# fenghansen/YOND_public

Hardware: AMD Instinct MI355X
Metric: Bayer megapixels/sec end-to-end (NLE+VST+denoise+iVST) (higher is better)
Workload: dtype f32 (3x3 convolutions: f32 operands as two f16 halves -- 22-23 significant bits -- on the f16 MFMA, 3 products per f32 product, f32 accumulate; per-layer error vs float64 asserted <= 2x the f32 direct kernel's and <= 2e-5 of max|ref| (tests/test_hip_conv.py; measured 1.3e-6 vs 1.5e-6), whole frame v

## Files before the change

### yond_public_amd/csrc/conv_split.hip

```cpp
#include "conv_split_kernel.h"

SPLIT_GROUP_K1S2(SPLIT_EXTERN)
SPLIT_GROUP_S1_64(SPLIT_EXTERN)
SPLIT_GROUP_S1_32(SPLIT_EXTERN)
SPLIT_GROUP_HALF(SPLIT_EXTERN)
SPLIT_GROUP_HALF128(SPLIT_EXTERN)
SPLIT_GROUP_HALF_TALL(SPLIT_EXTERN)
SPLIT_GROUP_FOLD(SPLIT_EXTERN)
SPLIT_GROUP_FOLD_S2(SPLIT_EXTERN)
SPLIT_GROUP_FOLD_K1(SPLIT_EXTERN)
SPLIT_GROUP_FOLD_NHWC(SPLIT_EXTERN)
SPLIT_GROUP_K1_D2(SPLIT_EXTERN)
SPLIT_GROUP_OSP(SPLIT_EXTERN)
SPLIT_GROUP_ISP(SPLIT_EXTERN)
SPLIT_GROUP_ISP_OSP(SPLIT_EXTERN)
SPLIT_GROUP_ISP_K1S2(SPLIT_EXTERN)
SPLIT_GROUP_K1_SUB2(SPLIT_EXTERN)
SPLIT_GROUP_WRES(SPLIT_EXTERN)
SPLIT_GROUP_D2(SPLIT_EXTERN)
SPLIT_GROUP_H_OSP(SPLIT_EXTERN)
SPLIT_GROUP_H_ISP_OSP(SPLIT_EXTERN)
SPLIT_GROUP_H_ISP_O4(SPLIT_EXTERN)
SPLIT_GROUP_H_K1S2(SPLIT_EXTERN)
SPLIT_GROUP_H_D2(SPLIT_EXTERN)
SPLIT_GROUP_H_SUB2(SPLIT_EXTERN)
SPLIT_GROUP_H128_OSP(SPLIT_EXTERN)
SPLIT_GROUP_H128_ISP_OSP(SPLIT_EXTERN)
// ... 180 lines not shown
            if (!isp || !d.src1) return YOND_EUNSUPPORTED;
            if (half128k1) return launch_split<1, 8, 128, 2, 1, 3, false, false, true, 2>(d, st);
            if (d.dst2) return launch_split<1, 8, 64, 2, 1, 3, false, false, true, 2, false, false, true>(d, st);
            if (tn == 64 && op4 && (long long)(d.Cout / 64) * ((d.Wo + 31) / 32) * ((d.Ho + 15) / 16) * d.N >= 256 && yond_exp_long("YOND_SPLIT_K1_TALL", 1) != 0)
                return launch_split<1, 16, 64, 4, 1, 2, false, false, true, 2>(d, st);
            return tn == 32 ? launch_split<1, 8, 32, 1, 1, 3, false, false, true, 2>(d, st) : launch_split<1, 8, 64, 2, 1, 3, false, false, true, 2>(d, st);
        }
        if (isp && tn == 64 && d.Wo <= 16 && d.src1 && !d.dst2 && yond_exp_long("YOND_SPLIT_FOLD", 1) != 0) {
            const int f = d.Wo <= 8 ? 4 : 2;
            const long long subs = (long long)d.N * ((d.Ho + 7) / 8) * ((d.Wo + 32 / f - 1) / (32 / f));
            const long long tiles_f = (long long)(d.Cout / 64) * ((subs + f - 1) / f), tiles = (long long)(d.Cout / 64) * ((d.Ho + 7) / 8) * d.N;
            const bool fits = (long long)d.H * d.W * (d.C0 > 4 * d.C1 ? d.C0 : 4 * d.C1) * 4 * f < (1LL << 31);
            if (fits && (tiles_f + 255) / 256 < (tiles + 255) / 256)
                return f == 2 ? launch_split<1, 8, 64, 2, 2, 3, false, false, true, 2, false, false, false, 2>(d, st) : launch_split<1, 8, 64, 2, 2, 3, false, false, true, 2, false, false, false, 4>(d, st);
        }
        if (isp && d.dst2) return launch_split<1, 8, 64, 2, 2, 3, false, false, true, 2, false, false, true>(d, st);
        if (isp) return tn == 32 ? launch_split<1, 8, 32, 1, 2, 3, false, false, true, 2>(d, st) : launch_split<1, 8, 64, 2, 2, 3, false, false, true, 2>(d, st);
        if (tn == 32) return launch_split<1, 8, 32, 1, 2, 3, false, false, true>(d, st);
        return launch_split<1, 8, 64, 2, 2, 3, false, false, true>(d, st);
    }
    if (d.stride == 2) {
        if (d.Ho != (d.H + 1) / 2 || d.Wo != (d.W + 1) / 2 || d.pre_act) return YOND_EINVAL;
        if (osp || ip4 || (op4 && d.res)) return YOND_EUNSUPPORTED;
        if (isp && parts == 2 && d.Wo <= 16 && !d.src1 && !d.res && yond_exp_long("YOND_SPLIT_FOLD", 1) != 0) {
            const int f = d.Wo <= 8 ? 4 : 2;
            const long long subs = (long long)d.N * ((d.Ho + 3) / 4) * ((d.Wo + 32 / f - 1) / (32 / f));
            const long long tiles_f = (long long)(d.Cout / 64) * ((subs + f - 1) / f), tiles = (long long)(d.Cout / 64) * ((d.Ho + 3) / 4) * d.N;
            const bool fits = (long long)d.H * d.W * d.C0 * 4 * f < (1LL << 31);
            if (fits && (tiles_f + 255) / 256 < (tiles + 255) / 256) {
                if (f == 2) return d.dst2 ? launch_split<2, 4, 64, 1, 2, 2, false, false, false, 2, false, false, true, 2>(d, st) : launch_split<2, 4, 64, 1, 2, 2, false, false, false, 2, false, false, false, 2>(d, st);
// ... 131 lines not shown
```

### yond_public_amd/csrc/conv_split_kernel.h

```cpp
#pragma once
#include "common.h"
#include <cstdlib>

typedef _Float16 f16x8 __attribute__((ext_vector_type(8)));
typedef _Float16 f16x4 __attribute__((ext_vector_type(4)));

#ifndef SPLIT_DBG
#define SPLIT_DBG 0
#endif
#if SPLIT_DBG
static __device__ unsigned long long g_split_dbg[2][64][12];
#ifdef SPLIT_DBG_READER
extern "C" int SPLIT_DBG_READER(unsigned long long* host) {
    return (int)hipMemcpyFromSymbol(host, HIP_SYMBOL(g_split_dbg), sizeof(g_split_dbg));
}
#endif
#define SDBG(slot)                                                                                  \
    do {                                                                                            \
        if (blockIdx.x == 0 && (wave == 0 || wave == 4) && lane == 0 && dbg_step < 64)              \
            g_split_dbg[wave >> 2][dbg_step][slot] = __builtin_readcyclecounter();                  \
    } while (0)
#else
#define SDBG(slot) do {} while (0)
#endif
// ... 57 lines not shown
    return n;
}
__device__ __forceinline__ float split_silu(float x) {
    return x * __builtin_amdgcn_rcpf(1.0f + __builtin_amdgcn_exp2f(x * -1.44269504088896341f));
}
template <int N>
__device__ __forceinline__ void split_barrier_keep_loads() { asm volatile("s_waitcnt vmcnt(%0) lgkmcnt(0)\n\ts_barrier" ::"n"(N) : "memory"); }

template <int STRIDE, int TH, int TN, int MW, int PARTS, int NWB, bool PRE, bool O4 = false, bool K1 = false, int ISPM = 0, bool OSP = false, bool S2 = false, bool D2 = false, int FOLD = 0, int NWAVE = 8, int ROLES = 0>
__global__ __launch_bounds__(64 * NWAVE, (NWAVE == 4 && STRIDE == 1) ? 2 : 1) void conv_split_kernel(const YondConvDesc d) {
    using C = SplitCfg<STRIDE, TH, TN, MW, PARTS, NWB, K1, FOLD, NWAVE, ROLES>;
    static_assert(!ROLES || (ISPM == 2 && !OSP && !O4 && !PRE), "role split: the register-staged split-plane input (stride 2)");
    static_assert(!FOLD || (!O4 && !S2 && ((!K1 && STRIDE == 1 && ISPM != 2 && OSP) || (STRIDE == 2 && (ISPM == 2 || (ISPM == 0 && !PRE && !D2))) || (K1 && ISPM == 2) || (!K1 && STRIDE == 1 && ISPM == 0 && !OSP && !PRE))),
                  "folded tiles: the split-plane data flow's kernels (3x3 stride 1: LDS-DMA or register-staged input, split-plane store; stride 2 and the decoder GEMM: register-staged split planes) "
                  "and the plain [N][H][W][C] 3x3 layer (training, UNetSeeInDark)");
    constexpr bool ISP = ISPM == 1, ISR = ISPM == 2;
    static_assert(ISPM == 0 || !PRE, "split-plane input: the producer applied the activation");
    static_assert(!OSP || (!O4 && !K1 && STRIDE == 1), "split-plane output: 3x3 stride-1 layers");
    static_assert(!S2 || (K1 && ISPM == 2 && TN == 64), "two sub-positions per tile: the decoder GEMM with register-staged split planes");
    static_assert(!D2 || (!OSP && !O4 && ((!K1 && STRIDE == 2) || (K1 && ISPM == 2 && !S2 && TN == 64))), "second output: the stride-2 layers and the decoder GEMM at split precision");
    constexpr int NACC = PARTS;
    constexpr int IPP = ISR ? 2 * PARTS : 4;
    constexpr int PIX_ITEMS = C::IH * C::IW * IPP;
    constexpr int NITEM = C::NPT * PIX_ITEMS;
    static_assert(!K1 || PIX_ITEMS % C::NTS == 0, "1x1 mode: whole chunks per pass of the staging threads");
    constexpr int NIN = ISP ? 0 : (NITEM + C::NTS - 1) / C::NTS;
    constexpr int NINA = NIN > 0 ? NIN : 1;
    constexpr int NDI = ISP ? C::NDI : 0;
    constexpr int KD = K1 ? PIX_ITEMS / C::NTS : NIN;
    constexpr int DPER = C::WPP / split_gcd(C::WPP, NWAVE);
    constexpr int NG = ISP ? (NDI < DPER ? NDI : DPER) : KD;
    constexpr int NOPS = C::NWT + NIN + NDI;
    constexpr int KEEP = (ISP || ROLES) ? (C::WAHEAD == 2 ? C::NWT_MIN : 0) : (C::WAHEAD == 2 ? NIN + C::NWT_MIN : NIN);
    extern __shared__ __attribute__((aligned(16))) float smem[];

    const int tid = threadIdx.x, lane = tid & 63, wave = tid >> 6;
    const int stid = ROLES ? tid - C::NTS : tid;
    const bool consumer = !ROLES || __builtin_amdgcn_readfirstlane(wave) < C::NWC;
    const int li = lane & 31, lh = lane >> 5;
    constexpr int FSW = FOLD ? 32 / FOLD : 32;
    const int fsub = FOLD ? li / FSW : 0, fcol = FOLD ? li % FSW : li, flds = (FOLD && !K1) ? li + (STRIDE == 2 ? 1 : 2) * fsub : li;
    const int rg = wave % C::RG, cg = wave / C::RG;

    const int nct = d.Cout / TN;
    const bool computes = d.Cout > 0;
    const int fnsx = (d.Wo + FSW - 1) / FSW, fnsy = (d.Ho + TH - 1) / TH;
    const int fper = fnsy * fnsx, fsubs = d.N * fper;
    struct FGeo { int n, oy0, ox0; };
// ... 18 lines not shown
    const int Cr = K1 ? d.Cout / 4 : d.Cout;
    const int cpb = S2 ? Cr / 32 : 1;
    auto k1_sp = [&](int ct, int cu) -> int {
        if constexpr (S2) return 2 * (ct / cpb) + ((cu >> 5) & 1);
        return cu / Cr;
    };
    auto k1_cb = [&](int ct, int cu) -> int {
        if constexpr (S2) return (ct % cpb) * 32 + (cu & 31);
        return cu % Cr;
    };
    const int my_sl = stid & (IPP - 1);
    const int my_plane = (my_sl >> 1) * PARTS * C::PLANE + (my_sl & 1) * 2;

    int in_lds[NINA];
#pragma unroll
    for (int k = 0; k < NIN; ++k) {
        const int it = stid + k * C::NTS;
        const int pt = it / PIX_ITEMS;
        const int pix = (it % PIX_ITEMS) / IPP;
        const int py = pix / C::IW, px = pix % C::IW;
        const int lp = (STRIDE == 2) ? py * C::TWP + (px & 1) * C::HALF + (px >> 1) : py * C::TWP + px;
        in_lds[k] = my_plane + (it < NITEM ? pt * 2 * PARTS * C::PLANE + lp * 4 : C::IH * C::TWP * 4);
        if constexpr (ISR) in_lds[k] = my_sl * C::PLANE + (it < NITEM ? pt * 2 * PARTS * C::PLANE + lp * 4 : C::IH * C::TWP * 4);
    }

    struct Tile {
        int ct, n, ox0, oy0;
        int fu0;
        int goff[NG];
        int goff1[K1 ? NG : 1];
    };
// ... 21 lines not shown
    auto tile_origin = [&](const Cur& c, Tile& T) {
        T.n = rev ? Neff - 1 - c.n : c.n;
        T.ct = c.ct;
        T.ox0 = (rev ? ntx - 1 - c.tx : c.tx) * 32;
        T.oy0 = (rev ? nty - 1 - c.ty : c.ty) * TH;
        T.fu0 = 0;
        if constexpr (FOLD != 0) {
            T.fu0 = FOLD * (rev ? ntx - 1 - c.tx : c.tx);
            const FGeo g = fold_geo(T.fu0);
            T.n = g.n; T.oy0 = g.oy0; T.ox0 = g.ox0;
        }
    };
    auto decode = [&](const Cur& c, Tile& T) {
        tile_origin(c, T);
        const int n = T.n;
        if constexpr (ISP) {
#pragma unroll
            for (int k = 0; k < NG; ++k) {
                const int sid = k * NWAVE + wave_s;
                const int q = (sid % C::WPP) * 64 + lane;
                const int py = q / C::TWP, rem = q % C::TWP;
                const int px = STRIDE == 2 ? 2 * (rem % C::HALF) + rem / C::HALF : rem;
                const bool valid = q < C::UPP && px < C::IW;
                int gy = K1 ? T.oy0 + py : T.oy0 * STRIDE - 1 + py, gx = K1 ? T.ox0 + px : T.ox0 * STRIDE - 1 + px;
                int nshift = 0;
                if constexpr (FOLD != 0) {
                    const int sb = px / C::FSUBW, lx = px - C::FSUBW * sb;
                    const FGeo g = fold_geo(T.fu0 + sb);
                    gy = g.oy0 >= d.Ho ? -1 : g.oy0 - 1 + py;
                    gx = g.ox0 - 1 + lx;
                    nshift = (g.n - T.n) * ((d.C0 / 16) * (2 * PARTS) * PS0 * 16);
// ... 26 lines not shown
                nb = d.in_fmt == YOND_FMT_PLANES4 ? nb + (g.n - n) * (d.C0 / 4) * d.H * d.W : g.n * d.H * d.W;
                ushift = (g.n - n) * (d.C0 / 16) * (2 * PARTS) * PS0;
            }
            const bool ok = it < NITEM && gy >= 0 && gy < d.H && gx >= 0 && gx < d.W;
            T.goff[k] = ok ? (nb + gy * d.W + gx) : -1;
            if constexpr (ISR) T.goff[k] = ok ? gy * d.W + gx + ushift : d.H * d.W;
            if constexpr (K1) {
                const int sp = k1_sp(T.ct, T.ct * TN);
                T.goff1[k] = ok ? ((n * 2 * d.H + 2 * gy + (sp >> 1)) * (2 * d.W) + 2 * gx + (sp & 1)) : -1;
                if constexpr (ISR) T.goff1[k] = ok ? (2 * gy + (sp >> 1)) * (2 * d.W) + 2 * gx + (sp & 1) + ushift1 : 4 * d.H * d.W;
            }
        }
        }
    };

    constexpr int NSET = ROLES ? 1 : (MW >= 3 || (STRIDE == 2 && PARTS == 1 && TN == 128)) ? 2 : 3;
    static_assert(NSET == 3 || C::WAHEAD == 1, "the two-set pipeline goes with two weight buffers");
    f32x4 vin[NSET][NINA];
    unsigned vin_ok[NSET] = {};
    YondRange amax;
    struct LoadSrc { const float* src[C::NPT]; int A[C::NPT], B[C::NPT]; bool hi[C::NPT]; int dx[C::NPT]; };
    const bool in_p4 = d.in_fmt == YOND_FMT_PLANES4;
    auto load_src = [&](int ch, int n) {
        LoadSrc L;
#pragma unroll
        for (int t = 0; t < C::NPT; ++t) {
            const int c0 = (ch * C::NPT + t) * C::KC;
            const bool second = c0 >= d.C0;
            int Cs = second ? d.C1 : d.C0, cc = second ? c0 - d.C0 : c0;
            L.src[t] = second ? d.src1 : d.src0;
            L.hi[t] = second && K1;
            L.dx[t] = 0;
// ... 72 lines not shown
        const int plane = sid / C::WPP, wv = sid - plane * C::WPP;
        const int pt = plane / (2 * PARTS), pl = plane - pt * (2 * PARTS);
        const bool hi = K1 && ((I.hi >> pt) & 1u);
        const unsigned lds0 = (unsigned)(uintptr_t)(__attribute__((address_space(3))) float*)ob;
        const unsigned lds_wave = __builtin_amdgcn_readfirstlane(lds0 + (unsigned)(plane * C::PLANE * 4 + wv * 1024));
        const char* b0 = I.base[0];
        if constexpr (C::NPT > 1) b0 = pt == 1 ? I.base[1] : (pt == 2 ? I.base[C::NPT - 1] : b0);
        const unsigned long long ga = (unsigned long long)(uintptr_t)(b0 + (size_t)pl * (size_t)(hi ? PS1 : PS0) * 16);
        const unsigned ga_lo = __builtin_amdgcn_readfirstlane((unsigned)ga), ga_hi = __builtin_amdgcn_readfirstlane((unsigned)(ga >> 32));
        const char* gb = (const char*)(uintptr_t)(((unsigned long long)ga_hi << 32) | ga_lo);
        int voff = T.goff[k % NG];
        if constexpr (K1) voff = hi ? T.goff1[k % NG] : voff;
        if (sid < C::NDS && voff >= 0)
            asm volatile("s_mov_b32 m0, %0\n\ts_nop 0\n\tglobal_load_lds_dwordx4 %1, %2" ::"s"(lds_wave), "v"(voff), "s"(gb) : "memory");
    };
    auto weight_src = [&](int ct, int ch) {
        const unsigned long long a = (unsigned long long)(uintptr_t)(d.wpk + ((size_t)ct * nchunk + ch) * C::W_FLOATS);
        const unsigned lo = __builtin_amdgcn_readfirstlane((unsigned)a), hi = __builtin_amdgcn_readfirstlane((unsigned)(a >> 32));
        return (const float*)(uintptr_t)(((unsigned long long)hi << 32) | lo);
    };
    constexpr int NE = 4 * NIN;
    auto stage_task = [&](auto pc, auto ec, float* ob) {
        constexpr int P = decltype(pc)::value;
        constexpr int e = decltype(ec)::value, k = e / 4, j = e % 4;
        if constexpr (ISR) {
            if constexpr (j == 3) *(f32x4*)(ob + in_lds[k]) = vin[P][k];
            return;
        }
        float x = vin[P][k][j];
        if (PRE) x = split_silu(x);
        vin[P][k][j] = ((vin_ok[P] >> k) & 1u) ? x : 0.0f;
        if constexpr (j == 3) {
            const f32x4 v = vin[P][k];
            amax.add(v);
            const f16x4 h = {(_Float16)v[0], (_Float16)v[1], (_Float16)v[2], (_Float16)v[3]};
            *(f16x4*)(ob + in_lds[k]) = h;
// ... 42 lines not shown
            constexpr int po = K1 ? dx * 2 * PARTS * C::PLANE : 0;
#pragma unroll
            for (int p = 0; p < PARTS; ++p) xr[q % XD][p] = *(lds_h8)(xb + po + p * C::PLANE + (r * C::TWP + xo) * 4);
        };
        auto loadW1 = [&](auto dc, auto yc) {
            constexpr int dx = decltype(dc)::value, dy = decltype(yc)::value;
            constexpr int tap = K1 ? dx : dy * 3 + dx;
#pragma unroll
            for (int nn = 0; nn < C::NW; ++nn)
#pragma unroll
                for (int p = 0; p < PARTS; ++p)
                    wt[dx % WS][dy][nn][p] = *(lds_h8)(wb + ((tap * 2 * PARTS + p) * TN + nn * 32) * 4);
        };
        auto loadW = [&](auto dc) { static_for<0, (K1 ? 1 : 3)>([&](auto yc) { loadW1(dc, yc); }); };
        loadW(IntC<0>{});
        loadX(IntC<0>{});
        loadX(IntC<1>{});
        static_for<0, NQ>([&](auto qc) {
            constexpr int q = decltype(qc)::value;
            constexpr int dx = q / R, r = q % R;
            constexpr bool wpre = !WINPLACE && (r == (R >= 4 ? R - 3 : 0) && dx < 2);
            constexpr int wdy = r - (MW - 1) * STRIDE;
            constexpr bool wrep = WINPLACE && dx < 2 && wdy >= 0 && wdy <= 2;
            if constexpr (q + 2 < NQ) loadX(IntC<q + 2>{});
            if constexpr (wpre) loadW(IntC<dx + 1>{});
            constexpr int nmf = (PARTS == 2 ? 3 : 1) * C::NW * (K1 ? 1 : split_pairs(MW, STRIDE, r));
#pragma unroll
            for (int a = 0; a < 3; ++a) {
                if (PARTS == 1 && a != 1) continue;
#pragma unroll
                for (int m = 0; m < MW; ++m) {
                    const int dy = K1 ? (m == r ? 0 : -1) : r - m * STRIDE;
                    if (dy < 0 || dy > 2) continue;
#pragma unroll
                    for (int nn = 0; nn < C::NW; ++nn)
                        acc[a == 1 ? 0 : 1][m][nn] = __builtin_amdgcn_mfma_f32_32x32x16_f16(
                            wt[dx % WS][dy][nn][a == 2 ? PARTS - 1 : 0], xr[q % XD][a == 0 ? PARTS - 1 : 0], acc[a == 1 ? 0 : 1][m][nn], 0, 0, 0);
                }
            }
            if constexpr (wrep) loadW1(IntC<dx + 1>{}, IntC<wdy>{});
            if constexpr (q == 0) { if (wave_hi) __builtin_amdgcn_s_setprio(1); }
            if constexpr (q == NQ / 2) { if (wave_hi) __builtin_amdgcn_s_setprio(0); }
            if constexpr (q == Q0 - 1 && !ROLES) prep();
            if constexpr (q == NQ / 4) SDBG(8);
            if constexpr (q == NQ / 2) SDBG(9);
            if constexpr (q == (3 * NQ) / 4) SDBG(10);
            constexpr int qq = q >= Q0 ? q - Q0 : 0;
            constexpr int NQO = (ISP && C::WAHEAD == 1) ? (NQW + 1) / 2 : NQW;
            constexpr int qo = qq < NQO ? qq : NQO;
            constexpr int o_lo = (q >= Q0 && !ROLES) ? (qo * NOPS + NQO - 1) / NQO : 0, o_hi = (q >= Q0 && !ROLES) ? ((qo + 1 < NQO ? qo + 1 : NQO) * NOPS + NQO - 1) / NQO : 0;
            static_for<o_lo, o_hi>([&](auto oc) {
                constexpr int o = decltype(oc)::value;
                if constexpr (ISP) {
                    if constexpr (o < NDI) issue_in_dma(IntC<o>{}, lt, is_s, ob);
                    else issue_dma(IntC<o - NDI>{}, wsrc_s, wnext);
                } else if constexpr (C::LOADS_FIRST) {
                    if constexpr (o < NIN) issue_load(fc, IntC<o>{}, lt, ls_s);
                    else issue_dma(IntC<o - NIN>{}, wsrc_s, wnext);
                } else {
                    if constexpr (o < C::NWT) issue_dma(IntC<o>{}, wsrc_s, wnext);
                    else issue_load(fc, IntC<o - C::NWT>{}, lt, ls_s);
                }
            });
            constexpr int e_lo = (q >= Q0 && !ROLES) ? qq * NE / NQW : 0, e_hi = (q >= Q0 && !ROLES) ? (qq + 1) * NE / NQW : 0;
            static_for<e_lo, e_hi>([&](auto ec) { stage_task(pc, ec, ob); });
            constexpr int nfin = (e_hi + 0) / 4 - (e_lo + 0) / 4;
            constexpr int nrd = (q + 2 < NQ ? PARTS : 0) + (wpre ? (K1 ? 1 : 3) * C::NW * PARTS : 0);
            if constexpr (nrd > 0) __builtin_amdgcn_sched_group_barrier(0x100, nrd, 0);
            constexpr int ntr = (!ISR && PRE) ? (e_hi - e_lo) * 2 : 0;
            constexpr int nvalu = ISR ? 0 : (e_hi - e_lo) * (PRE ? 5 : 2) + nfin * (PARTS == 2 ? 22 : 6);
            constexpr int vpm = (nvalu + nmf - 1) / nmf;
#pragma unroll
            for (int i = 0; i < nmf; ++i) {
                __builtin_amdgcn_sched_group_barrier(0x008, 1, 0);
                if ((i * ntr) / nmf != ((i + 1) * ntr) / nmf) __builtin_amdgcn_sched_group_barrier(0x400, 1, 0);
                if constexpr (vpm > 0) __builtin_amdgcn_sched_group_barrier(0x002, vpm, 0);
            }
            if constexpr (wrep) __builtin_amdgcn_sched_group_barrier(0x100, C::NW * PARTS, 0);
            if constexpr (nfin > 0) __builtin_amdgcn_sched_group_barrier(0x200, ISR ? nfin : nfin * PARTS, 0);
        });
    };

    const float slope_eff = d.post_act == 2 ? d.slope : 1.0f;
    const bool silu_out = d.post_act == 1;
    constexpr int EPS = 36;
    constexpr int EP_FLOATS = NWAVE * 32 * EPS;
    constexpr bool EP_IN_W = TN >= 64 && !K1;
    constexpr bool EP_FIT = STRIDE == 1 && (C::EP_OWN || EP_FLOATS <= (EP_IN_W ? C::W_FLOATS : C::IN_FLOATS));
    f32x4 pes[C::NW], pet[C::NW];
    auto epi_prefetch = [&](const Tile& T) __attribute__((always_inline)) {
        const int u = lane & 7;
#pragma unroll
        for (int nn = 0; nn < C::NW; ++nn) {
// ... 289 lines not shown
    auto epilogue_direct = [&](const Tile& T) __attribute__((always_inline)) {
        const FGeo lg = lane_geo(T);
        const int ox = lg.ox0;
        const bool col_ok = ox < d.Wo;
        const bool out_p4 = d.out_fmt == YOND_FMT_PLANES4;
        const int Hout = K1 ? 2 * d.Ho : d.Ho, Wout = K1 ? 2 * d.Wo : d.Wo;
#pragma unroll
        for (int nn = 0; nn < C::NW; ++nn) {
            const int cfull = T.ct * TN + (cg * C::NW + nn) * 32 + 4 * lh;
            const int sp = K1 ? k1_sp(T.ct, cfull) : 0, cbase = K1 ? k1_cb(T.ct, cfull) : cfull;
            const int eoff = (d.ebatch ? lg.n * Cr : 0) + cbase;
            f32x4 es[4], et[4];
#pragma unroll
            for (int g = 0; g < 4; ++g) {
                const f32x4 one = {1.0f, 1.0f, 1.0f, 1.0f}, zero4 = {0.0f, 0.0f, 0.0f, 0.0f};
                es[g] = d.escale ? *(const f32x4*)(d.escale + eoff + 8 * g) : one;
                et[g] = d.eshift ? *(const f32x4*)(d.eshift + eoff + 8 * g) : zero4;
            }
            f32x4 rr[MW][4];
#pragma unroll
            for (int m = 0; m < MW; ++m) {
                const int oy = lg.oy0 + rg * MW + m;
                const bool ok = col_ok && oy < d.Ho;
                const long long off = ok ? ((long long)(lg.n * d.Ho + oy) * d.Wo + ox) * d.Cout + cbase : 0;
#pragma unroll
                for (int g = 0; g < 4; ++g) {
                    const f32x4 z = {0.0f, 0.0f, 0.0f, 0.0f};
                    rr[m][g] = (d.res && !K1) ? *(const f32x4*)(d.res + off + (ok ? 8 * g : 0)) : z;
                }
            }
#pragma unroll
            for (int m = 0; m < MW; ++m) {
// ... 66 lines not shown
    int lt_tile = -1;
    decode(cs, cur);
    zero_acc();
    float* ibuf = smem;
    float* obuf = smem + C::IN_FLOATS;
    float* w0 = smem + 2 * C::IN_FLOATS;
    float* w1 = w0 + C::W_FLOATS;
    float* w2 = w1 + (NWB == 3 ? C::W_FLOATS : 0);
    auto ct_of = [&](Cur c, int fallback) { return c.tile < total ? c.ct : fallback; };
    auto tile_for = [&](Cur c) {
        if (c.tile < total && c.tile != lt_tile) { decode(c, lt); lt_tile = c.tile; }
    };
    auto load_all = [&](auto pc, Cur c) {
        tile_for(c);
        const LoadSrc L = load_src(c.ch, lt.n);
        static_for<0, NIN>([&](auto kc) { issue_load(pc, kc, lt, L); });
    };
    auto dma_in_all = [&](Cur c, float* ob) {
        tile_for(c);
        const InSrc I = in_src(c.ch, lt.n);
        static_for<0, NDI>([&](auto kc) { issue_in_dma(kc, lt, I, ob); });
    };
    auto dma_all = [&](Cur c, float* wb) {
        const float* ws = weight_src(ct_of(c, cur.ct), c.ch);
        static_for<0, C::NWT>([&](auto kc) { issue_dma(kc, ws, wb); });
    };
    const Cur c1 = adv(cs), c2 = adv(c1);
    if constexpr (!ISP) { if (!ROLES || !consumer) load_all(IntC<0>{}, cs); }
    Cur cl, cw;
    if constexpr (ISP) {
        dma_in_all(cs, ibuf);
        dma_all(cs, w0);
        if constexpr (C::WAHEAD == 2) dma_all(c1, w1);
        cl = c1;
        cw = C::WAHEAD == 2 ? c2 : c1;
        split_barrier_keep_loads<C::WAHEAD == 2 ? C::NWT_MIN : 0>();
    } else if constexpr (ROLES != 0) {
        if (!consumer) {
            dma_all(cs, w0);
            write_in(IntC<0>{}, ibuf);
        }
        cl = c1;
        cw = c1;
        split_barrier_keep_loads<0>();
    } else if constexpr (NSET == 2) {
        dma_all(cs, w0);
        write_in(IntC<0>{}, ibuf);
        load_all(IntC<1>{}, c1);
        cl = c2;
        cw = c1;
        split_barrier_keep_loads<NIN>();
// ... 3 lines not shown
            dma_all(cs, w0);
            write_in(IntC<0>{}, ibuf);
            load_all(IntC<2>{}, c2);
            dma_all(c1, w1);
        } else {
            dma_all(cs, w0);
            load_all(IntC<1>{}, c1);
            write_in(IntC<0>{}, ibuf);
            if constexpr (C::WAHEAD == 2) dma_all(c1, w1);
            load_all(IntC<2>{}, c2);
        }
        cl = adv(c2);
        cw = C::WAHEAD == 2 ? c2 : c1;
        split_barrier_keep_loads<C::WAHEAD == 2 ? NIN + C::NWT_MIN : 2 * NIN>();
    }
    auto step = [&](auto sc) __attribute__((always_inline)) -> bool {
        constexpr int S = decltype(sc)::value;
        SDBG(0);
        const bool last_ch = (cs.ch + 1 == nchunk);
        const Cur cn = adv(cs);
        if constexpr (EP_FIT || OSP) {
            if (last_ch) {
                epi_prefetch(cur);
                res_prefetch(cur);
                res4_prefetch(cur);
            }
        }
        auto prep = [&]() __attribute__((always_inline)) {
            tile_for(cl);
            if constexpr (ISP) is_s = in_src(cl.ch, lt.n);
            else ls_s = load_src(cl.ch, lt.n);
            wsrc_s = weight_src(ct_of(cw, cur.ct), cw.ch);
        };
        SDBG(1);
        if constexpr (ROLES != 0) {
            if (consumer) {
                if (computes) mfma_stage(IntC<0>{}, IntC<0>{}, ibuf, w0, obuf, w1, lt, prep);
            } else {
                prep();
                static_for<0, C::NWT>([&](auto kc) { issue_dma(kc, wsrc_s, w1); });
                static_for<0, NIN>([&](auto kc) { issue_load(IntC<0>{}, kc, lt, ls_s); });
                write_in(IntC<0>{}, obuf);
            }
        } else if (computes) mfma_stage(IntC<(S + 1) % NSET>{}, IntC<S>{}, ibuf, w0, obuf, C::WAHEAD == 2 ? w2 : w1, lt, prep);
        SDBG(2);
        SDBG(3);
        split_barrier_keep_loads<KEEP>();
        SDBG(4);
        if (last_ch) {
            if (computes && consumer) {
                if constexpr (OSP) {
                    const int flags = (d.res ? 1 : 0) | (d.escale ? 2 : 0) | (d.eshift ? 4 : 0);
                    if (flags == 6 && d.post_act == 1) epilogue_sp(IntC<6>{}, IntC<1>{}, cur);
                    else if (ORP && flags == 7 && d.post_act == 0) {
                        if constexpr (ORP) epilogue_sp(IntC<7>{}, IntC<0>{}, cur);
                    } else if (flags == 4 && d.post_act == 2) epilogue_sp(IntC<4>{}, IntC<2>{}, cur);
                    else
                        static_for<0, 8>([&](auto fcx) __attribute__((always_inline)) {
                            if constexpr (ORP || (decltype(fcx)::value & 1) == 0) {
                                if (flags == decltype(fcx)::value) epilogue_sp(fcx, IntC<-1>{}, cur);
                            }
                        });
                } else if (K1 && (FOLD != 0 || D2 || d.out_fmt == YOND_FMT_PLANES4)) {
                    epilogue_direct(cur);
                } else if constexpr (EP_FIT) {
                    float* scr = C::EP_OWN ? smem + C::EP_OFF : (EP_IN_W ? w0 : ibuf);
                    const int flags = (d.res ? 1 : 0) | (d.escale ? 2 : 0) | (d.eshift ? 4 : 0);
                    if (flags == 7 && d.post_act == 0) epilogue(IntC<7>{}, IntC<0>{}, cur, scr);
                    else if (flags == 6 && d.post_act == 1) epilogue(IntC<6>{}, IntC<1>{}, cur, scr);
                    else if (flags == 4 && d.post_act == 2) epilogue(IntC<4>{}, IntC<2>{}, cur, scr);
                    else if (flags == 4 && d.post_act == 0) epilogue(IntC<4>{}, IntC<0>{}, cur, scr);
                    else
                        static_for<0, 8>([&](auto fcx) __attribute__((always_inline)) {
                            if (flags == decltype(fcx)::value) epilogue(fcx, IntC<-1>{}, cur, scr);
                        });
                } else {
                    epilogue_direct(cur);
                }
            }
            SDBG(6);
            if constexpr (EP_FIT && !OSP) asm volatile("s_waitcnt lgkmcnt(0)\n\ts_barrier" ::: "memory");
            SDBG(7);
            zero_acc();
            if (cn.tile < total) {
                tile_origin(cn, cur);
            }
        }
        SDBG(5);
        ++dbg_step;
        wskip = wres;
        if (cn.tile >= total) return false;
        cs = cn;
        cl = adv(cl);
        cw = adv(cw);
        float* t = ibuf;
        ibuf = obuf;
        obuf = t;
        t = w0;
        w0 = w1;
        w1 = NWB == 3 ? w2 : t;
        w2 = t;
        return true;
    };
    while (true) {
        if (!step(IntC<0>{})) break;
        if (!step(IntC<1>{})) break;
        if constexpr (NSET == 3) {
            if (!step(IntC<2>{})) break;
        }
    }
    asm volatile("s_waitcnt vmcnt(0)" ::: "memory");
    if (d.status && !amax.at_most(65504.0f)) atomicOr(d.status, YOND_STATUS_HALF_OVERFLOW);
    if (clk_on) {
        atomicAdd(d.clk, __builtin_amdgcn_s_memtime() - clk_c0);
        atomicAdd(d.clk + 1, __builtin_amdgcn_s_memrealtime() - clk_r0);
    }
}

template <int STRIDE, int TH, int TN, int MW, int PARTS, int NWB, bool PRE, bool O4 = false, bool K1 = false, int ISP = 0, bool OSP = false, bool S2 = false, bool D2 = false, int FOLD = 0, int NWAVE = 8, int ROLES = 0>
int launch_split(const YondConvDesc& d, hipStream_t st) {
    using C = SplitCfg<STRIDE, TH, TN, MW, PARTS, NWB, K1, FOLD, NWAVE, ROLES>;
    static_assert(C::SMEM_BYTES <= 160 * 1024, "LDS budget");
    static bool attr_set = false;
// ... 41 lines not shown
#define SPLIT_GROUP_ISP(X)                                                                              \
    X(1, 12, 64, 3, 2, 2, false, false, false, true, false) X(1, 8, 64, 2, 2, 3, false, false, false, true, false) \
    X(1, 16, 32, 2, 2, 3, false, true, false, true, false) X(1, 16, 32, 2, 2, 3, false, false, false, true, false)
#define SPLIT_GROUP_ISP_OSP(X)                                                                          \
    X(1, 12, 64, 3, 2, 2, false, false, false, true, true) X(1, 8, 64, 2, 2, 3, false, false, false, true, true) \
    X(1, 16, 32, 2, 2, 3, false, false, false, true, true)
#define SPLIT_GROUP_ISP_K1S2(X)                                                                         \
    X(1, 8, 32, 1, 2, 3, false, false, true, 2, false) X(1, 8, 64, 2, 2, 3, false, false, true, 2, false) \
    X(2, 4, 64, 1, 2, 2, false, false, false, 2, false)
#define SPLIT_GROUP_K1_SUB2(X) X(1, 8, 64, 2, 2, 3, false, false, true, 2, false, true)
#define SPLIT_GROUP_FOLD(X)                                                                             \
    X(1, 4, 64, 1, 2, 3, false, false, false, true, true, false, false, 2) X(1, 4, 64, 1, 2, 3, true, false, false, false, true, false, false, 2)         \
    X(1, 4, 64, 1, 2, 3, false, false, false, true, true, false, false, 4) X(1, 4, 64, 1, 2, 3, true, false, false, false, true, false, false, 4)
#define SPLIT_GROUP_FOLD_NHWC(X) X(1, 4, 64, 1, 2, 3, false, false, false, 0, false, false, false, 2) X(1, 4, 64, 1, 2, 3, false, false, false, 0, false, false, false, 4)
#define SPLIT_GROUP_K1_D2(X) X(1, 8, 64, 2, 2, 3, false, false, true, 2, false, false, true)
#define SPLIT_GROUP_FOLD_K1(X) X(1, 8, 64, 2, 2, 3, false, false, true, 2, false, false, false, 2) X(1, 8, 64, 2, 2, 3, false, false, true, 2, false, false, false, 4)
#define SPLIT_GROUP_FOLD_S2(X)                                                                          \
    X(2, 4, 64, 1, 2, 2, false, false, false, 2, false, false, true, 2) X(2, 4, 64, 1, 2, 2, false, false, false, 2, false, false, false, 2)            \
    X(2, 4, 64, 1, 2, 2, false, false, false, 2, false, false, true, 4) X(2, 4, 64, 1, 2, 2, false, false, false, 2, false, false, false, 4)            \
    X(2, 4, 64, 1, 2, 2, false, false, false, 0, false, false, false, 2) X(2, 4, 64, 1, 2, 2, false, false, false, 0, false, false, false, 4)
#define SPLIT_GROUP_D2(X) X(2, 4, 64, 1, 2, 2, false, false, false, 2, false, false, true)
#define SPLIT_GROUP_WRES(X)                                                                             \
    X(1, 16, 32, 2, 2, 2, true, false, false, false, true) X(1, 16, 32, 2, 2, 2, false, false, false, true, true) \
    X(1, 16, 32, 2, 2, 2, false, true, false, true, false)
#define SPLIT_GROUP_H_OSP(X)                                                                            \
    X(1, 12, 64, 3, 1, 2, true, false, false, false, true) X(1, 8, 64, 2, 1, 3, true, false, false, false, true) \
    X(1, 16, 32, 2, 1, 3, true, false, false, false, true)
#define SPLIT_GROUP_H_ISP_OSP(X)                                                                        \
    X(1, 12, 64, 3, 1, 2, false, false, false, true, true) X(1, 8, 64, 2, 1, 3, false, false, false, true, true) \
    X(1, 16, 32, 2, 1, 3, false, false, false, true, true)
// ... 25 lines not shown
```

Baseline: 2649.

## Add register-direct input mode for split-precision 1x1 decoder GEMM

Adds a new input mode (ISPM=3) for the 64-wide 1x1 split-precision kernel. It loads the split-plane input fragments straight from global memory into registers in MFMA operand layout, skipping LDS staging. The main loop becomes two-stage with prefetch one tile ahead, and it now runs by default through an env-gated dispatch. In exchange it uses more vector registers and may issue less coalesced global loads, and the loop and epilogue control flow gets more complex.

```diff
diff --git a/yond_public_amd/csrc/conv_split.hip b/yond_public_amd/csrc/conv_split.hip
--- a/yond_public_amd/csrc/conv_split.hip
+++ b/yond_public_amd/csrc/conv_split.hip
@@ -11,6 +11,7 @@
 SPLIT_GROUP_FOLD_K1(SPLIT_EXTERN)
 SPLIT_GROUP_FOLD_NHWC(SPLIT_EXTERN)
 SPLIT_GROUP_K1_D2(SPLIT_EXTERN)
+SPLIT_GROUP_K1_DIRECT(SPLIT_EXTERN)
 SPLIT_GROUP_OSP(SPLIT_EXTERN)
 SPLIT_GROUP_ISP(SPLIT_EXTERN)
 SPLIT_GROUP_ISP_OSP(SPLIT_EXTERN)
@@ -221,6 +222,8 @@
             if (fits && (tiles_f + 255) / 256 < (tiles + 255) / 256)
                 return f == 2 ? launch_split<1, 8, 64, 2, 2, 3, false, false, true, 2, false, false, false, 2>(d, st) : launch_split<1, 8, 64, 2, 2, 3, false, false, true, 2, false, false, false, 4>(d, st);
         }
+        if (isp && tn == 64 && yond_exp_long("YOND_SPLIT_K1_DIRECT", 1) != 0)
+            return d.dst2 ? launch_split<1, 8, 64, 2, 2, 3, false, false, true, 3, false, false, true>(d, st) : launch_split<1, 8, 64, 2, 2, 3, false, false, true, 3>(d, st);
         if (isp && d.dst2) return launch_split<1, 8, 64, 2, 2, 3, false, false, true, 2, false, false, true>(d, st);
         if (isp) return tn == 32 ? launch_split<1, 8, 32, 1, 2, 3, false, false, true, 2>(d, st) : launch_split<1, 8, 64, 2, 2, 3, false, false, true, 2>(d, st);
         if (tn == 32) return launch_split<1, 8, 32, 1, 2, 3, false, false, true>(d, st);
diff --git a/yond_public_amd/csrc/conv_split_k1_direct.hip b/yond_public_amd/csrc/conv_split_k1_direct.hip
--- /dev/null
+++ b/yond_public_amd/csrc/conv_split_k1_direct.hip
@@ -0,0 +1,3 @@
+#include "conv_split_kernel.h"
+
+SPLIT_GROUP_K1_DIRECT(SPLIT_INSTANTIATE)
diff --git a/yond_public_amd/csrc/conv_split_kernel.h b/yond_public_amd/csrc/conv_split_kernel.h
--- a/yond_public_amd/csrc/conv_split_kernel.h
+++ b/yond_public_amd/csrc/conv_split_kernel.h
@@ -95,24 +95,25 @@
     static_assert(!FOLD || (!O4 && !S2 && ((!K1 && STRIDE == 1 && ISPM != 2 && OSP) || (STRIDE == 2 && (ISPM == 2 || (ISPM == 0 && !PRE && !D2))) || (K1 && ISPM == 2) || (!K1 && STRIDE == 1 && ISPM == 0 && !OSP && !PRE))),
                   "folded tiles: the split-plane data flow's kernels (3x3 stride 1: LDS-DMA or register-staged input, split-plane store; stride 2 and the decoder GEMM: register-staged split planes) "
                   "and the plain [N][H][W][C] 3x3 layer (training, UNetSeeInDark)");
-    constexpr bool ISP = ISPM == 1, ISR = ISPM == 2;
+    constexpr bool ISP = ISPM == 1, ISR = ISPM == 2, ISD = ISPM == 3;
+    static_assert(!ISD || (K1 && PARTS == 2 && TN == 64 && MW == 2 && NWB == 3 && !S2 && FOLD == 0 && NWAVE == 8 && !ROLES && !O4 && !OSP), "register-direct input: the 64-wide unfolded decoder GEMM");
     static_assert(ISPM == 0 || !PRE, "split-plane input: the producer applied the activation");
     static_assert(!OSP || (!O4 && !K1 && STRIDE == 1), "split-plane output: 3x3 stride-1 layers");
     static_assert(!S2 || (K1 && ISPM == 2 && TN == 64), "two sub-positions per tile: the decoder GEMM with register-staged split planes");
-    static_assert(!D2 || (!OSP && !O4 && ((!K1 && STRIDE == 2) || (K1 && ISPM == 2 && !S2 && TN == 64))), "second output: the stride-2 layers and the decoder GEMM at split precision");
+    static_assert(!D2 || (!OSP && !O4 && ((!K1 && STRIDE == 2) || (K1 && (ISPM == 2 || ISPM == 3) && !S2 && TN == 64))), "second output: the stride-2 layers and the decoder GEMM at split precision");
     constexpr int NACC = PARTS;
     constexpr int IPP = ISR ? 2 * PARTS : 4;
     constexpr int PIX_ITEMS = C::IH * C::IW * IPP;
     constexpr int NITEM = C::NPT * PIX_ITEMS;
     static_assert(!K1 || PIX_ITEMS % C::NTS == 0, "1x1 mode: whole chunks per pass of the staging threads");
-    constexpr int NIN = ISP ? 0 : (NITEM + C::NTS - 1) / C::NTS;
+    constexpr int NIN = ISP ? 0 : ISD ? C::NPT * MW * PARTS : (NITEM + C::NTS - 1) / C::NTS;
     constexpr int NINA = NIN > 0 ? NIN : 1;
     constexpr int NDI = ISP ? C::NDI : 0;
-    constexpr int KD = K1 ? PIX_ITEMS / C::NTS : NIN;
+    constexpr int KD = ISD ? MW : K1 ? PIX_ITEMS / C::NTS : NIN;
     constexpr int DPER = C::WPP / split_gcd(C::WPP, NWAVE);
     constexpr int NG = ISP ? (NDI < DPER ? NDI : DPER) : KD;
     constexpr int NOPS = C::NWT + NIN + NDI;
-    constexpr int KEEP = (ISP || ROLES) ? (C::WAHEAD == 2 ? C::NWT_MIN : 0) : (C::WAHEAD == 2 ? NIN + C::NWT_MIN : NIN);
+    constexpr int KEEP = ISD ? 2 * NIN + C::NWT_MIN : (ISP || ROLES) ? (C::WAHEAD == 2 ? C::NWT_MIN : 0) : (C::WAHEAD == 2 ? NIN + C::NWT_MIN : NIN);
     extern __shared__ __attribute__((aligned(16))) float smem[];
 
     const int tid = threadIdx.x, lane = tid & 63, wave = tid >> 6;
@@ -161,7 +162,7 @@
 
     int in_lds[NINA];
 #pragma unroll
-    for (int k = 0; k < NIN; ++k) {
+    for (int k = 0; k < (ISD ? 0 : NIN); ++k) {
         const int it = stid + k * C::NTS;
         const int pt = it / PIX_ITEMS;
         const int pix = (it % PIX_ITEMS) / IPP;
@@ -213,7 +214,16 @@
     auto decode = [&](const Cur& c, Tile& T) {
         tile_origin(c, T);
         const int n = T.n;
-        if constexpr (ISP) {
+        if constexpr (ISD) {
+            const int sp = k1_sp(T.ct, T.ct * TN);
+#pragma unroll
+            for (int m = 0; m < MW; ++m) {
+                const int gy = T.oy0 + rg * MW + m, gx = T.ox0 + li;
+                const bool in = gy < d.H && gx < d.W;
+                T.goff[m] = (in ? gy * d.W + gx : d.H * d.W) + lh * PARTS * PS0;
+                T.goff1[m] = (in ? (2 * gy + (sp >> 1)) * (2 * d.W) + 2 * gx + (sp & 1) : 4 * d.H * d.W) + lh * PARTS * PS1;
+            }
+        } else if constexpr (ISP) {
 #pragma unroll
             for (int k = 0; k < NG; ++k) {
                 const int sid = k * NWAVE + wave_s;
@@ -270,8 +280,8 @@
         }
     };
 
-    constexpr int NSET = ROLES ? 1 : (MW >= 3 || (STRIDE == 2 && PARTS == 1 && TN == 128)) ? 2 : 3;
-    static_assert(NSET == 3 || C::WAHEAD == 1, "the two-set pipeline goes with two weight buffers");
+    constexpr int NSET = ROLES ? 1 : (ISD || MW >= 3 || (STRIDE == 2 && PARTS == 1 && TN == 128)) ? 2 : 3;
+    static_assert(NSET == 3 || C::WAHEAD == 1 || ISD, "the two-set pipeline goes with two weight buffers");
     f32x4 vin[NSET][NINA];
     unsigned vin_ok[NSET] = {};
     YondRange amax;
@@ -374,12 +384,19 @@
         if (sid < C::NDS && voff >= 0)
             asm volatile("s_mov_b32 m0, %0\n\ts_nop 0\n\tglobal_load_lds_dwordx4 %1, %2" ::"s"(lds_wave), "v"(voff), "s"(gb) : "memory");
     };
+    auto issue_frag = [&](auto pc, auto kc, const Tile& T, const InSrc& I) {
+        constexpr int P = decltype(pc)::value, k = decltype(kc)::value;
+        constexpr int t = k / (MW * PARTS), m = (k / PARTS) % MW, p = k % PARTS;
+        const bool hi = (I.hi >> t) & 1u;
+        const unsigned u = (unsigned)((hi ? T.goff1[m % KD] : T.goff[m % KD]) + p * (hi ? PS1 : PS0));
+        vin[P][k] = *(const __attribute__((address_space(1))) f32x4*)(uintptr_t)(I.base[t] + (size_t)(u * 16u));
+    };
     auto weight_src = [&](int ct, int ch) {
         const unsigned long long a = (unsigned long long)(uintptr_t)(d.wpk + ((size_t)ct * nchunk + ch) * C::W_FLOATS);
         const unsigned lo = __builtin_amdgcn_readfirstlane((unsigned)a), hi = __builtin_amdgcn_readfirstlane((unsigned)(a >> 32));
         return (const float*)(uintptr_t)(((unsigned long long)hi << 32) | lo);
     };
-    constexpr int NE = 4 * NIN;
+    constexpr int NE = ISD ? 0 : 4 * NIN;
     auto stage_task = [&](auto pc, auto ec, float* ob) {
         constexpr int P = decltype(pc)::value;
         constexpr int e = decltype(ec)::value, k = e / 4, j = e % 4;
@@ -452,15 +469,18 @@
         };
         auto loadW = [&](auto dc) { static_for<0, (K1 ? 1 : 3)>([&](auto yc) { loadW1(dc, yc); }); };
         loadW(IntC<0>{});
-        loadX(IntC<0>{});
-        loadX(IntC<1>{});
+        if constexpr (!ISD) {
+            loadX(IntC<0>{});
+            loadX(IntC<1>{});
+        }
         static_for<0, NQ>([&](auto qc) {
             constexpr int q = decltype(qc)::value;
             constexpr int dx = q / R, r = q % R;
             constexpr bool wpre = !WINPLACE && (r == (R >= 4 ? R - 3 : 0) && dx < 2);
             constexpr int wdy = r - (MW - 1) * STRIDE;
             constexpr bool wrep = WINPLACE && dx < 2 && wdy >= 0 && wdy <= 2;
-            if constexpr (q + 2 < NQ) loadX(IntC<q + 2>{});
+            if constexpr (q + 2 < NQ && !ISD) loadX(IntC<q + 2>{});
+            constexpr int F = decltype(fc)::value;
             if constexpr (wpre) loadW(IntC<dx + 1>{});
             constexpr int nmf = (PARTS == 2 ? 3 : 1) * C::NW * (K1 ? 1 : split_pairs(MW, STRIDE, r));
 #pragma unroll
@@ -473,7 +493,9 @@
 #pragma unroll
                     for (int nn = 0; nn < C::NW; ++nn)
                         acc[a == 1 ? 0 : 1][m][nn] = __builtin_amdgcn_mfma_f32_32x32x16_f16(
-                            wt[dx % WS][dy][nn][a == 2 ? PARTS - 1 : 0], xr[q % XD][a == 0 ? PARTS - 1 : 0], acc[a == 1 ? 0 : 1][m][nn], 0, 0, 0);
+                            wt[dx % WS][dy][nn][a == 2 ? PARTS - 1 : 0],
+                            ISD ? __builtin_bit_cast(f16x8, vin[ISD ? F : 0][ISD ? q * PARTS + (a == 0 ? PARTS - 1 : 0) : 0]) : xr[q % XD][a == 0 ? PARTS - 1 : 0],
+                            acc[a == 1 ? 0 : 1][m][nn], 0, 0, 0);
                 }
             }
             if constexpr (wrep) loadW1(IntC<dx + 1>{}, IntC<wdy>{});
@@ -487,7 +509,10 @@
             constexpr int NQO = (ISP && C::WAHEAD == 1) ? (NQW + 1) / 2 : NQW;
             constexpr int qo = qq < NQO ? qq : NQO;
             constexpr int o_lo = (q >= Q0 && !ROLES) ? (qo * NOPS + NQO - 1) / NQO : 0, o_hi = (q >= Q0 && !ROLES) ? ((qo + 1 < NQO ? qo + 1 : NQO) * NOPS + NQO - 1) / NQO : 0;
-            static_for<o_lo, o_hi>([&](auto oc) {
+            constexpr int f_lo = (ISD && q >= Q0) ? q : 0, f_hi = (ISD && q >= Q0 - 1) ? q + 1 : 0;
+            if constexpr (ISD && q == Q0 - 1) static_for<0, C::NWT>([&](auto kc) { issue_dma(kc, wsrc_s, wnext); });
+            static_for<f_lo * PARTS, f_hi * PARTS>([&](auto kc) { issue_frag(fc, kc, lt, is_s); });
+            static_for<(ISD ? 0 : o_lo), (ISD ? 0 : o_hi)>([&](auto oc) {
                 constexpr int o = decltype(oc)::value;
                 if constexpr (ISP) {
                     if constexpr (o < NDI) issue_in_dma(IntC<o>{}, lt, is_s, ob);
@@ -503,7 +528,7 @@
             constexpr int e_lo = (q >= Q0 && !ROLES) ? qq * NE / NQW : 0, e_hi = (q >= Q0 && !ROLES) ? (qq + 1) * NE / NQW : 0;
             static_for<e_lo, e_hi>([&](auto ec) { stage_task(pc, ec, ob); });
             constexpr int nfin = (e_hi + 0) / 4 - (e_lo + 0) / 4;
-            constexpr int nrd = (q + 2 < NQ ? PARTS : 0) + (wpre ? (K1 ? 1 : 3) * C::NW * PARTS : 0);
+            constexpr int nrd = (q + 2 < NQ && !ISD ? PARTS : 0) + (wpre ? (K1 ? 1 : 3) * C::NW * PARTS : 0);
             if constexpr (nrd > 0) __builtin_amdgcn_sched_group_barrier(0x100, nrd, 0);
             constexpr int ntr = (!ISR && PRE) ? (e_hi - e_lo) * 2 : 0;
             constexpr int nvalu = ISR ? 0 : (e_hi - e_lo) * (PRE ? 5 : 2) + nfin * (PARTS == 2 ? 22 : 6);
@@ -515,6 +540,7 @@
                 if constexpr (vpm > 0) __builtin_amdgcn_sched_group_barrier(0x002, vpm, 0);
             }
             if constexpr (wrep) __builtin_amdgcn_sched_group_barrier(0x100, C::NW * PARTS, 0);
+            if constexpr (ISD && f_hi > f_lo) __builtin_amdgcn_sched_group_barrier(0x020, (f_hi - f_lo) * PARTS, 0);
             if constexpr (nfin > 0) __builtin_amdgcn_sched_group_barrier(0x200, ISR ? nfin : nfin * PARTS, 0);
         });
     };
@@ -834,8 +860,21 @@
 #pragma unroll
             for (int g = 0; g < 4; ++g) {
                 const f32x4 one = {1.0f, 1.0f, 1.0f, 1.0f}, zero4 = {0.0f, 0.0f, 0.0f, 0.0f};
+                if constexpr (ISD) {
+                    es[g] = *(const f32x4*)(d.escale ? d.escale + eoff + 8 * g : d.wpk);
+                    et[g] = *(const f32x4*)(d.eshift ? d.eshift + eoff + 8 * g : d.wpk);
+                    continue;
+                }
                 es[g] = d.escale ? *(const f32x4*)(d.escale + eoff + 8 * g) : one;
                 et[g] = d.eshift ? *(const f32x4*)(d.eshift + eoff + 8 * g) : zero4;
+            }
+            if constexpr (ISD) {
+#pragma unroll
+                for (int g = 0; g < 4; ++g) {
+                    const f32x4 one = {1.0f, 1.0f, 1.0f, 1.0f}, zero4 = {0.0f, 0.0f, 0.0f, 0.0f};
+                    es[g] = d.escale ? es[g] : one;
+                    et[g] = d.eshift ? et[g] : zero4;
+                }
             }
             f32x4 rr[MW][4];
 #pragma unroll
@@ -932,7 +971,12 @@
     auto load_all = [&](auto pc, Cur c) {
         tile_for(c);
         const LoadSrc L = load_src(c.ch, lt.n);
-        static_for<0, NIN>([&](auto kc) { issue_load(pc, kc, lt, L); });
+        static_for<0, (ISD ? 0 : NIN)>([&](auto kc) { issue_load(pc, kc, lt, L); });
+    };
+    auto frag_all = [&](auto pc, Cur c) {
+        tile_for(c);
+        const InSrc I = in_src(c.ch, lt.n);
+        static_for<0, (ISD ? NIN : 0)>([&](auto kc) { issue_frag(pc, kc, lt, I); });
     };
     auto dma_in_all = [&](Cur c, float* ob) {
         tile_for(c);
@@ -944,7 +988,7 @@
         static_for<0, C::NWT>([&](auto kc) { issue_dma(kc, ws, wb); });
     };
     const Cur c1 = adv(cs), c2 = adv(c1);
-    if constexpr (!ISP) { if (!ROLES || !consumer) load_all(IntC<0>{}, cs); }
+    if constexpr (!ISP && !ISD) { if (!ROLES || !consumer) load_all(IntC<0>{}, cs); }
     Cur cl, cw;
     if constexpr (ISP) {
         dma_in_all(cs, ibuf);
@@ -953,6 +997,14 @@
         cl = c1;
         cw = C::WAHEAD == 2 ? c2 : c1;
         split_barrier_keep_loads<C::WAHEAD == 2 ? C::NWT_MIN : 0>();
+    } else if constexpr (ISD) {
+        dma_all(cs, w0);
+        frag_all(IntC<0>{}, cs);
+        frag_all(IntC<1>{}, c1);
+        dma_all(c1, w1);
+        cl = c2;
+        cw = c2;
+        split_barrier_keep_loads<NIN + C::NWT_MIN>();
     } else if constexpr (ROLES != 0) {
         if (!consumer) {
             dma_all(cs, w0);
@@ -986,7 +1038,7 @@
         cw = C::WAHEAD == 2 ? c2 : c1;
         split_barrier_keep_loads<C::WAHEAD == 2 ? NIN + C::NWT_MIN : 2 * NIN>();
     }
-    auto step = [&](auto sc) __attribute__((always_inline)) -> bool {
+    auto step = [&](auto sc, bool live) __attribute__((always_inline)) -> bool {
         constexpr int S = decltype(sc)::value;
         SDBG(0);
         const bool last_ch = (cs.ch + 1 == nchunk);
@@ -1000,7 +1052,7 @@
         }
         auto prep = [&]() __attribute__((always_inline)) {
             tile_for(cl);
-            if constexpr (ISP) is_s = in_src(cl.ch, lt.n);
+            if constexpr (ISP || ISD) is_s = in_src(cl.ch, lt.n);
             else ls_s = load_src(cl.ch, lt.n);
             wsrc_s = weight_src(ct_of(cw, cur.ct), cw.ch);
         };
@@ -1014,12 +1066,12 @@
                 static_for<0, NIN>([&](auto kc) { issue_load(IntC<0>{}, kc, lt, ls_s); });
                 write_in(IntC<0>{}, obuf);
             }
-        } else if (computes) mfma_stage(IntC<(S + 1) % NSET>{}, IntC<S>{}, ibuf, w0, obuf, C::WAHEAD == 2 ? w2 : w1, lt, prep);
+        } else if (ISD || computes) mfma_stage(IntC<(S + 1) % NSET>{}, IntC<S>{}, ibuf, w0, obuf, C::WAHEAD == 2 ? w2 : w1, lt, prep);
         SDBG(2);
         SDBG(3);
         split_barrier_keep_loads<KEEP>();
         SDBG(4);
-        if (last_ch) {
+        if (last_ch && live) {
             if (computes && consumer) {
                 if constexpr (OSP) {
                     const int flags = (d.res ? 1 : 0) | (d.escale ? 2 : 0) | (d.eshift ? 4 : 0);
@@ -1033,8 +1085,9 @@
                                 if (flags == decltype(fcx)::value) epilogue_sp(fcx, IntC<-1>{}, cur);
                             }
                         });
-                } else if (K1 && (FOLD != 0 || D2 || d.out_fmt == YOND_FMT_PLANES4)) {
+                } else if (K1 && (ISD || FOLD != 0 || D2 || d.out_fmt == YOND_FMT_PLANES4)) {
                     epilogue_direct(cur);
+                    if constexpr (ISD) __builtin_amdgcn_s_waitcnt(0x0F70);
                 } else if constexpr (EP_FIT) {
                     float* scr = C::EP_OWN ? smem + C::EP_OFF : (EP_IN_W ? w0 : ibuf);
                     const int flags = (d.res ? 1 : 0) | (d.escale ? 2 : 0) | (d.eshift ? 4 : 0);
@@ -1051,7 +1104,7 @@
                 }
             }
             SDBG(6);
-            if constexpr (EP_FIT && !OSP) asm volatile("s_waitcnt lgkmcnt(0)\n\ts_barrier" ::: "memory");
+            if constexpr (EP_FIT && !OSP && !ISD) asm volatile("s_waitcnt lgkmcnt(0)\n\ts_barrier" ::: "memory");
             SDBG(7);
             zero_acc();
             if (cn.tile < total) {
@@ -1061,7 +1114,7 @@
         SDBG(5);
         ++dbg_step;
         wskip = wres;
-        if (cn.tile >= total) return false;
+        if constexpr (!ISD) { if (cn.tile >= total) return false; }
         cs = cn;
         cl = adv(cl);
         cw = adv(cw);
@@ -1072,13 +1125,20 @@
         w0 = w1;
         w1 = NWB == 3 ? w2 : t;
         w2 = t;
-        return true;
-    };
+        return ISD ? cn.tile < total : true;
+    };
+    if constexpr (ISD) {
+        bool go = true;
+        while (go) {
+            const bool a = step(IntC<0>{}, true);
+            go = step(IntC<1>{}, a) && a;
+        }
+    } else
     while (true) {
-        if (!step(IntC<0>{})) break;
-        if (!step(IntC<1>{})) break;
+        if (!step(IntC<0>{}, true)) break;
+        if (!step(IntC<1>{}, true)) break;
         if constexpr (NSET == 3) {
-            if (!step(IntC<2>{})) break;
+            if (!step(IntC<2>{}, true)) break;
         }
     }
     asm volatile("s_waitcnt vmcnt(0)" ::: "memory");
@@ -1150,6 +1210,7 @@
     X(1, 4, 64, 1, 2, 3, false, false, false, true, true, false, false, 4) X(1, 4, 64, 1, 2, 3, true, false, false, false, true, false, false, 4)
 #define SPLIT_GROUP_FOLD_NHWC(X) X(1, 4, 64, 1, 2, 3, false, false, false, 0, false, false, false, 2) X(1, 4, 64, 1, 2, 3, false, false, false, 0, false, false, false, 4)
 #define SPLIT_GROUP_K1_D2(X) X(1, 8, 64, 2, 2, 3, false, false, true, 2, false, false, true)
+#define SPLIT_GROUP_K1_DIRECT(X) X(1, 8, 64, 2, 2, 3, false, false, true, 3, false) X(1, 8, 64, 2, 2, 3, false, false, true, 3, false, false, true)
 #define SPLIT_GROUP_FOLD_K1(X) X(1, 8, 64, 2, 2, 3, false, false, true, 2, false, false, false, 2) X(1, 8, 64, 2, 2, 3, false, false, true, 2, false, false, false, 4)
 #define SPLIT_GROUP_FOLD_S2(X)                                                                          \
     X(2, 4, 64, 1, 2, 2, false, false, false, 2, false, false, true, 2) X(2, 4, 64, 1, 2, 2, false, false, false, 2, false, false, false, 2)            \
```

Result: no change. 2652 (median of 5 runs) (+0.1%).
